# awkrail/svpc

Hardware: AMD Instinct MI355X
Metric: train steps/sec (vivt, batch=16, clip_seq=12) (higher is better)
Workload: dtype bf16x3; 1 GPU; MODEL_TYPE=vivt train step: N=16 videos/GPU x S=12 clips x Lv=100 frames x F=3072, Lt=22, D=768, H=12, L=6 (enc+step-enc+dec), V=951, A=384, E=10; dropout .1/.1/.4; fwd+bwd+allreduce+clip+BertAdam; mode=bf16x3, global_batch=16, parallelism=dp1, launch=hipGraph replay, gpus_requested=1

## Files before the change

include/svpc_hip.h:

```cpp
#ifndef SVPC_HIP_H
#define SVPC_HIP_H
#include <stddef.h>
#ifdef __cplusplus
extern "C" {
#endif

typedef struct ihipStream_t* svpc_stream_t;
typedef unsigned long long svpc_u64;

#define SVPC_ACT_NONE 0
#define SVPC_ACT_RELU 1
#define SVPC_ACT_GELU 2
#define SVPC_ACT_SIGMOID 3

const char* svpc_last_error(void);
int svpc_abi_version(void);

int svpc_ln_fwd(const float* x, const int* src_rows, const float* res, const float* gamma, const float* beta, float* y,
                float* mean, float* rstd, int R, int D, float eps, float p_pre, unsigned site_pre, float p_post,
                unsigned site_post, const svpc_u64* seed, const float* add1, int mod1, const float* add2, const int* idx2,
                svpc_stream_t stream);
int svpc_ln_fwd_t(const void* x, int x_dt, const int* src_rows, const void* res, const float* gamma, const float* beta, void* y,
                  int y_dt, float* mean, float* rstd, int R, int D, float eps, float p_pre, unsigned site_pre, float p_post,
                  unsigned site_post, const svpc_u64* seed, const float* add1, int mod1, const float* add2, const int* idx2,
// ... 67 lines not shown
int svpc_gemm_l32_preferred(int a_kc, int b_kc, int lda, int ldb, int M, int N, int K);
int svpc_gemm_l32(const float* A, int lda, int a_kc, const float* B, int ldb, int b_kc, float* C, int ldc, float* Z, int M, int N, int K,
                  const float* bias, int act, float p_drop, unsigned site, const svpc_u64* seed, int accumulate, float* workspace,
                  size_t workspace_bytes, svpc_stream_t stream);
int svpc_gemm_l32_r(const float* A, int lda, int a_kc, const float* B, int ldb, int b_kc, float* C, int ldc, float* Z, const float* R, int M,
                    int N, int K, const float* bias, int act, float p_drop, unsigned site, const svpc_u64* seed, int accumulate,
                    float* workspace, size_t workspace_bytes, svpc_stream_t stream);
int svpc_gemm_l32_rg(const float* A, int lda, int a_kc, const float* B, int ldb, int b_kc, float* C, int ldc, const float* R, const float* G,
                     int gact, int M, int N, int K, int accumulate, float* workspace, size_t workspace_bytes, svpc_stream_t stream);
int svpc_gemm_l32_x3(const float* A, int lda, int a_kc, const float* B, int ldb, int b_kc, float* C, int ldc, float* Z, const float* R, int M,
                     int N, int K, const float* bias, int act, float p_drop, unsigned site, const svpc_u64* seed, int accumulate,
                     float* workspace, size_t workspace_bytes, svpc_stream_t stream);
typedef struct svpc_gemm_problem { const float* A; const float* B; float* C; int M, N, K, lda, ldb, ldc; } svpc_gemm_problem;
int svpc_gemm_group(const svpc_gemm_problem* problems, int n, int a_kc, int b_kc, int accumulate, svpc_stream_t stream);
int svpc_gemm_group_x3(const svpc_gemm_problem* problems, int n, int a_kc, int b_kc, int accumulate, svpc_stream_t stream);
typedef struct svpc_wgrad_problem {
    const float* dz; const float* x; float* dw; float* db;
    int n_out, n_in, rows, ld_dz, ld_x, ld_dw;
} svpc_wgrad_problem;
int svpc_gemm_group_wgrad_max(void);
int svpc_gemm_group_wgrad_bf16_p8_ok(const void* problems, int n);
int svpc_gemm_group_wgrad_bf16_p8(const void* problems, int n, float* workspace, size_t workspace_bytes, svpc_stream_t stream);
int svpc_gemm_group_wgrad_bf16(const svpc_wgrad_problem* problems, int n, svpc_stream_t stream);
int svpc_gemm_group_wgrad_bf16_ws(const svpc_wgrad_problem* problems, int n, float* workspace, size_t workspace_bytes,
                                  svpc_stream_t stream);
int svpc_gemm_group_wgrad(const svpc_wgrad_problem* problems, int n, svpc_stream_t stream);
int svpc_act_bwd(const float* dy, const float* aux, float* dz, size_t n, int act, float p, unsigned site, const svpc_u64* seed,
                 svpc_stream_t stream);

int svpc_act_bwd_t(const void* dy, const void* aux, void* dz, int dt, size_t n, int act, float p, unsigned site, const svpc_u64* seed,
// ... 114 lines not shown
int svpc_ptr_mix_ce_bwd(const float* logits, const float* g, const float* pi, const int* labels, const int* row_c,
                        const int* row_vid, const int* csr_off, const int* csr_ent, const int* csr_id, const float* csr_w,
                        const float* P, const float* dP_ext, const float* dloss, float* dlogits, float* dg, float* dpi, int R, int V,
                        int c_max, int e_max, float smoothing, const float* row_w, svpc_stream_t stream);

int svpc_gumbel_noise(float* out, size_t n, unsigned site, const svpc_u64* seed, svpc_stream_t stream);
int svpc_gumbel_fwd(const float* P, const float* noise, const int* row_c, const float* emb, float* bow, int* idx, float* stats, int R,
                    int c_max, int V, int W, float tau, svpc_stream_t stream);
int svpc_gumbel_bwd(const float* P, const float* noise, const int* row_c, const float* stats, const float* dy, float* dP, int R,
                    int c_max, int V, float tau, svpc_stream_t stream);
int svpc_gumbel_emb_grad(const float* dbow, const int* idx, const float* stats, float* demb, int R, int V, int W,
                         svpc_stream_t stream);

int svpc_rownorm_fwd(const float* a, float* y, int R, int C, int mode, svpc_stream_t stream);
int svpc_rownorm_bwd(const float* dy, const float* y, const float* a, float* da, int R, int C, int mode, svpc_stream_t stream);
int svpc_span_mean_fwd(const float* x, const int* starts, const int* lens, const float* w, const float* add, const int* add_idx,
                       float* out, int G, int D, svpc_stream_t stream);
int svpc_span_mean_bwd(const float* dout, const int* starts, const int* lens, const float* w, float* dx, int G, int D,
                       svpc_stream_t stream);
int svpc_scatter_add_rows(const float* dx, const int* idx, float* dtable, int R, int D, int pad_row, svpc_stream_t stream);
int svpc_bce_rows_fwd(const float* p, const float* y, const int* widths, float* out, int R, int C, svpc_stream_t stream);
int svpc_bce_rows_bwd(const float* dout, const float* p, const float* y, const int* widths, float* dp, int R, int C,
                      svpc_stream_t stream);
int svpc_asl_rows_fwd(const float* p, const float* y, const float* active, float* out, int R, int C, float gneg, float gpos,
                      float clip, float eps, svpc_stream_t stream);
int svpc_asl_rows_bwd(const float* dout, const float* p, const float* y, const float* active, float* dp, int R, int C, float gneg,
                      float gpos, float clip, float eps, svpc_stream_t stream);
int svpc_loss_tail_ws_floats(int n_cap, int R);
int svpc_loss_tail_fwd(const float* cap_rows, int n_cap, const float* e_p, const float* align, const int* widths, int R, int Ce,
                       const float* a_p, const float* act, int Ca, const float* r_e, const float* r_a, float lambda, float gneg,
// ... 178 lines not shown
```

svpc_amd/csrc/elementwise.hip:

```cpp
#include "common.h"

template <typename T>
__global__ __launch_bounds__(256) void act_bwd_kernel(const T* __restrict__ dy, const T* __restrict__ aux,
                                                      T* __restrict__ dz, size_t n, int act, float p, uint32_t site,
                                                      const u64* __restrict__ seed_ptr) {
    const u64 seed = p > 0.f ? seed_ptr[0] : 0ull;
    const float ik = p > 0.f ? 1.0f / (1.0f - p) : 1.0f;
    for (size_t i = (size_t)blockIdx.x * 256 + threadIdx.x; i < n; i += (size_t)gridDim.x * 256) {
        float g = (float)dy[i];
        if (p > 0.f) g *= drop_scale(seed, site, i, p, ik);
        const float a = (float)aux[i];
        if (act == ACT_RELU) g = a > 0.f ? g : 0.f;
        else if (act == ACT_GELU) g *= gelu_erf_grad(a);
        else if (act == ACT_SIGMOID) g *= a * (1.0f - a);
        dz[i] = (T)g;
    }
}

__global__ __launch_bounds__(256) void act_bwd_bf16x8_kernel(const uint4* __restrict__ dy, const uint4* __restrict__ aux, uint4* __restrict__ dz,
                                                             size_t n8, int act, float p, uint32_t site, const u64* __restrict__ seed_ptr) {
    const u64 seed = p > 0.f ? seed_ptr[0] : 0ull;
    const float ik = p > 0.f ? 1.0f / (1.0f - p) : 1.0f;
    for (size_t q = (size_t)blockIdx.x * 256 + threadIdx.x; q < n8; q += (size_t)gridDim.x * 256) {
        const uint4 gv = dy[q], av = aux[q];
// ... 85 lines not shown
    }
}
__global__ __launch_bounds__(256) void rownorm_bwd_kernel(const float* __restrict__ dy, const float* __restrict__ y,
                                                          const float* __restrict__ a, float* __restrict__ da, int R, int C, int mode) {
    const int lane = threadIdx.x & 63, r = __builtin_amdgcn_readfirstlane(blockIdx.x * 4 + (threadIdx.x >> 6));
    if (r >= R) return;
    const size_t o = (size_t)r * C;
    float dot = 0.f, s = 0.f;
    for (int c = lane; c < C; c += 64) { dot += dy[o + c] * y[o + c]; if (mode == 0) s += a[o + c]; }
    dot = wave_sum(dot);
    if (mode == 0) {
        s = 1.0f / wave_sum(s);
        for (int c = lane; c < C; c += 64) da[o + c] = (dy[o + c] - dot) * s;
    } else {
        for (int c = lane; c < C; c += 64) da[o + c] = y[o + c] * (dy[o + c] - dot);
    }
}

__global__ __launch_bounds__(256) void span_mean_fwd_kernel(const float* __restrict__ x, const int* __restrict__ starts,
                                                            const int* __restrict__ lens, const float* __restrict__ w,
                                                            const float* __restrict__ add, const int* __restrict__ add_idx,
                                                            float* __restrict__ out, int G, int D) {
    const int g = blockIdx.x;
    const int s = starts[g], l = lens[g];
    for (int c = threadIdx.x; c < D; c += 256) {
        float acc = 0.f, wsum = 0.f;
        for (int r0 = 0; r0 < l; r0 += 8) {
            float xv[8], wv[8];
#pragma unroll
            for (int u = 0; u < 8; ++u) xv[u] = x[(size_t)(s + min(r0 + u, l - 1)) * D + c];
// ... 717 lines not shown
int svpc_fill_from(float* x, size_t n, const float* v, hipStream_t s) {
    if (n == 0) return 0;
    hipLaunchKernelGGL(fill_kernel, dim3(grid1d(n)), dim3(256), 0, s, x, n, v);
    return svpc_check_launch("fill_from");
}
int svpc_rownorm_fwd(const float* a, float* y, int R, int C, int mode, hipStream_t s) {
    if (R == 0) return 0;
    hipLaunchKernelGGL(rownorm_fwd_kernel, dim3(ceil_div(R, 4)), dim3(256), 0, s, a, y, R, C, mode);
    return svpc_check_launch("rownorm_fwd");
}
int svpc_rownorm_bwd(const float* dy, const float* y, const float* a, float* da, int R, int C, int mode, hipStream_t s) {
    if (R == 0) return 0;
    hipLaunchKernelGGL(rownorm_bwd_kernel, dim3(ceil_div(R, 4)), dim3(256), 0, s, dy, y, a, da, R, C, mode);
    return svpc_check_launch("rownorm_bwd");
}
int svpc_span_mean_fwd(const float* x, const int* starts, const int* lens, const float* w, const float* add, const int* add_idx,
                       float* out, int G, int D, hipStream_t s) {
    if (G == 0) return 0;
    hipLaunchKernelGGL(span_mean_fwd_kernel, dim3(G), dim3(256), 0, s, x, starts, lens, w, add, add_idx, out, G, D);
    return svpc_check_launch("span_mean_fwd");
}
int svpc_span_mean_bwd(const float* dout, const int* starts, const int* lens, const float* w, float* dx, int G, int D,
                       hipStream_t s) {
    if (G == 0) return 0;
    hipLaunchKernelGGL(span_mean_bwd_kernel, dim3(G), dim3(256), 0, s, dout, starts, lens, w, dx, G, D);
    return svpc_check_launch("span_mean_bwd");
}
int svpc_scatter_add_rows(const float* dx, const int* idx, float* dtable, int R, int D, int pad_row, hipStream_t s) {
    if (R == 0) return 0;
    hipLaunchKernelGGL(scatter_add_rows_kernel, dim3(R), dim3(256), 0, s, dx, idx, dtable, R, D, pad_row);
// ... 214 lines not shown
```

svpc_amd/csrc/gemm_l32.hip:

```cpp
#include "gemm_common.h"
#include <stdlib.h>

typedef __bf16 bf16x8 __attribute__((ext_vector_type(8)));
typedef const void __attribute__((address_space(1))) * l32_gptr;
typedef void __attribute__((address_space(3))) * l32_lptr;

constexpr int L32_BK = 32;
__device__ __attribute__((aligned(16))) const float l32_zeros[4] = {0.f, 0.f, 0.f, 0.f};

template <int N> __device__ __forceinline__ void l32_wait_vmcnt() { asm volatile("s_waitcnt vmcnt(%0)" ::"n"(N) : "memory"); }

template <int R, bool KC>
__device__ __forceinline__ const float* l32_src(const float* P, int ld, int m0, int rows, int k0, int j, int lane) {
    if (KC) {
        const int row = 8 * j + (lane >> 3), pos = lane & 7;
        const int c = pos ^ ((row >> 1) & 7);
        const int gr = min(m0 + row, rows - 1);
        return P + (size_t)gr * ld + k0 + 4 * c;
    } else {
        constexpr int CPR = R / 4;
        const int krow = j * (64 / CPR) + lane / CPR, c = lane % CPR;
        const int gm = min(m0 + 4 * c, rows - 4);
        return P + (size_t)(k0 + krow) * ld + gm;
    }
// ... 407 lines not shown

template <bool A_KC, bool B_KC, bool X3 = false>
static int gemm_group_go(const GemmGroupArgs& g, int tiles, hipStream_t stream) {
    constexpr int LDS = 4 * 2 * 2 * 64 * L32_BK * 4;
    static bool attr_set = false;
    if (!attr_set) {
        hipError_t e = hipFuncSetAttribute(reinterpret_cast<const void*>(&gemm_group_kernel<A_KC, B_KC, X3>),
                                           hipFuncAttributeMaxDynamicSharedMemorySize, LDS);
        if (e != hipSuccess) { svpc_set_error("gemm_group: cannot raise the dynamic LDS limit"); return (int)e; }
        attr_set = true;
    }
    hipLaunchKernelGGL((gemm_group_kernel<A_KC, B_KC, X3>), dim3(tiles), dim3(256), LDS, stream, g);
    return svpc_check_launch("gemm_group");
}

template <bool B_KC, int NW, bool X3 = false>
__device__ __forceinline__ void skinny_partials(float (*part)[16][64], const float* __restrict__ arow, const float* __restrict__ brow,
                                                int ldb, int K) {
    constexpr int BATCH = NW == 8 ? 10 : 12;
    const int lane = threadIdx.x & 63, wave = __builtin_amdgcn_readfirstlane(threadIdx.x >> 6);
    const int nsteps = K >> 4;
    floatx16 acc;
#pragma unroll
    for (int e = 0; e < 16; ++e) acc[e] = 0.f;
    for (int s0 = wave; s0 < nsteps; s0 += NW * BATCH) {
        float4 av[BATCH][2];
        float bv[BATCH][8];
#pragma unroll
        for (int u = 0; u < BATCH; ++u) {
            const int s = min(s0 + NW * u, nsteps - 1);
            const float* ap = arow + 16 * s;
            av[u][0] = *reinterpret_cast<const float4*>(ap);
            av[u][1] = *reinterpret_cast<const float4*>(ap + 4);
            if (B_KC) {
                const float* bp = brow + 16 * s;
                const float4 b0 = *reinterpret_cast<const float4*>(bp), b1 = *reinterpret_cast<const float4*>(bp + 4);
                bv[u][0] = b0.x; bv[u][1] = b0.y; bv[u][2] = b0.z; bv[u][3] = b0.w;
                bv[u][4] = b1.x; bv[u][5] = b1.y; bv[u][6] = b1.z; bv[u][7] = b1.w;
            } else {
                const float* bp = brow + (size_t)(16 * s) * ldb;
#pragma unroll
                for (int j = 0; j < 8; ++j) bv[u][j] = bp[(size_t)j * ldb];
            }
        }
#pragma unroll
        for (int u = 0; u < BATCH; ++u) {
            const int s = s0 + NW * u;
            if (s < nsteps) {
// ... 52 lines not shown
                                                          float* __restrict__ C, int ldc, int M, int N, int K, Epi epi, int tiles_n, int ts) {
    __shared__ float part[4][16][64];
    const int tm = blockIdx.x / tiles_n, tn = blockIdx.x - tm * tiles_n;
    skinny_tile<B_KC, 4, X3>(part, A, lda, B, ldb, C, ldc, M, N, K, epi, tm, tn, ts);
}
template <int NW, bool X3 = false, bool B_KC = true>
__global__ __launch_bounds__(64 * NW) void gemm_group_skinny_kernel(GemmGroupArgs g) {
    __shared__ float part[NW][16][64];
    int pi = 0;
    while (pi + 1 < g.n && (int)blockIdx.x >= g.p[pi + 1].tile0) ++pi;
    const GemmProb& q = g.p[pi];
    const int tile = blockIdx.x - q.tile0;
    const int tm = tile / q.tiles_n, tn = tile - tm * q.tiles_n;
    Epi epi{nullptr, ACT_NONE, 0.f, 0u, nullptr, g.accumulate, nullptr};
    skinny_tile<B_KC, NW, X3>(part, q.A, q.lda, q.B, q.ldb, q.C, q.ldc, q.M, q.N, q.K, epi, tm, tn);
}

struct LstmStep {
    const float* h_prev[2]; const float* c_prev[2]; const float* w_hh[2]; const float* gx[2]; const int* rows[2]; const float* active;
    float* h[2]; float* c[2]; float* gates[2]; int N, D;
};
template <bool X3>
__global__ __launch_bounds__(256) void lstm_pair_step_fwd_kernel(LstmStep a) {
    __shared__ float part[4][16][64];
    const int z = blockIdx.y, u0 = blockIdx.x * 8, m0 = blockIdx.z * 32;
    const int lane = threadIdx.x & 63, r = lane & 31, hh = lane >> 5;
    const int N = a.N, D = a.D;
    const float* arow = a.h_prev[z] + (size_t)min(m0 + r, N - 1) * D + 8 * hh;
    const float* brow = a.w_hh[z] + (size_t)((r >> 3) * D + u0 + (r & 7)) * D + 8 * hh;
    const int row = threadIdx.x >> 3, j = threadIdx.x & 7, n = m0 + row;
// ... 64 lines not shown
    if (!a_kc && (M % 4 != 0)) return 0;
    if (!b_kc && (N % 4 != 0)) return 0;
    return 1;
}

int svpc_gemm_l32_preferred(int a_kc, int b_kc, int lda, int ldb, int M, int N, int K) {
    if (!svpc_gemm_l32_supported(a_kc, b_kc, lda, ldb, M, N, K)) return 0;
    const int t128 = ceil_div(M, 128) * ceil_div(N, 128), t64 = ceil_div(M, 64) * ceil_div(N, 64);
    static int env_w = -1;
    if (env_w < 0) { const char* e = getenv("SVPC_L32_WAVESPLIT"); env_w = e ? atoi(e) : 1; }
    if (K % L32_BK != 0) return (t128 <= 300) ? 1 : 0;
    if (env_w && t64 <= 256 && K >= 4 * L32_BK && t64 * 4 >= 32) return 1;
    return (t128 <= 300 && K < 2048) ? 1 : 0;
}

struct HostWgradProblem { const float* dz; const float* x; float* dw; float* db; int n_out, n_in, rows, ld_dz, ld_x, ld_dw; };

int svpc_gemm_group_wgrad_max(void) { return GROUP_MAX; }

static int gemm_group_x(const void* problems, int n, int a_kc, int b_kc, int accumulate, int x3, hipStream_t stream) {
    if (n == 0) return 0;
    SVPC_REQUIRE(n > 0 && n <= GEMM_GROUP_MAX, "gemm_group: 1..32 problems per launch");
    const HostGemmProblem* hp = reinterpret_cast<const HostGemmProblem*>(problems);
    GemmGroupArgs g{};
    g.n = n; g.accumulate = accumulate;
    int tiles = 0;
    static int env_skinny = -1;
    if (env_skinny < 0) { const char* e = getenv("SVPC_L32_SKINNY"); env_skinny = e ? atoi(e) : 1; }
    bool skinny = env_skinny && a_kc;
    if (!b_kc && x3) skinny = false;
// ... 105 lines not shown
                           workspace_bytes, stream);
}
}
static int gemm_l32_x(const float* A, int lda, int a_kc, const float* B, int ldb, int b_kc, float* C, int ldc, float* Z, const float* R,
                      const float* G, int gact, int M, int N, int K, const float* bias, int act, float p_drop, unsigned site, const u64* seed,
                      int accumulate, float* workspace, size_t workspace_bytes, int x3, hipStream_t stream) {
    if (M == 0 || N == 0) return 0;
    SVPC_REQUIRE(svpc_gemm_l32_supported(a_kc, b_kc, lda, ldb, M, N, K) && ((((uintptr_t)A) | ((uintptr_t)B)) & 15) == 0,
                 "gemm_l32: needs K % 32 == 0 (or both operands k-contiguous and K % 4 == 0) and 16-byte aligned fp32 rows");
    SVPC_REQUIRE(p_drop <= 0.f || seed != nullptr, "gemm: dropout needs a seed pointer");
    Epi epi{bias, act, p_drop, site, seed, accumulate, Z, R, G, gact};
    static int env_tile = -1, env_split = -1;
    const int remap = gemm_remap_env();
    if (env_tile < 0) { const char* e = getenv("SVPC_L32_TILE"); env_tile = e ? atoi(e) : 0; }
    if (env_split < 0) { const char* e = getenv("SVPC_L32_SPLITK"); env_split = e ? atoi(e) : 0; }
    static int env_skinny = -1;
    if (env_skinny < 0) { const char* e = getenv("SVPC_L32_SKINNY"); env_skinny = e ? atoi(e) : 1; }
    static int skinny_m = -1;
    if (skinny_m < 0) { const char* e = getenv("SVPC_L32_SKINNY_M"); skinny_m = e ? atoi(e) : 256; }
    if (env_skinny && a_kc && M <= skinny_m && N >= 32 && (K & 15) == 0 && (lda & 3) == 0 && (!b_kc || (ldb & 3) == 0)) {
        static int env_ts = -1;
        if (env_ts < 0) { const char* e = getenv("SVPC_L32_SKINNY_TS"); env_ts = e ? atoi(e) : 24; }
        const int t24 = ceil_div(M, 24) * ceil_div(N, 24), t32 = ceil_div(M, 32) * ceil_div(N, 32);
        const int ts = (env_ts == 24 && t24 <= 256 && t32 < t24 && t32 > 64) ? 24 : 32;
        const int tn_ = ceil_div(N, ts);
        dim3 grids(ceil_div(M, ts) * tn_);
        if (x3) {
            if (b_kc) hipLaunchKernelGGL((gemm_skinny_kernel<true, true>), grids, dim3(256), 0, stream, A, lda, B, ldb, C, ldc, M, N, K, epi, tn_, ts);
            else hipLaunchKernelGGL((gemm_skinny_kernel<false, true>), grids, dim3(256), 0, stream, A, lda, B, ldb, C, ldc, M, N, K, epi, tn_, ts);
        } else if (b_kc) hipLaunchKernelGGL((gemm_skinny_kernel<true, false>), grids, dim3(256), 0, stream, A, lda, B, ldb, C, ldc, M, N, K, epi, tn_, ts);
        else hipLaunchKernelGGL((gemm_skinny_kernel<false, false>), grids, dim3(256), 0, stream, A, lda, B, ldb, C, ldc, M, N, K, epi, tn_, ts);
        return svpc_check_launch("gemm_skinny");
    }
    const int t128 = ceil_div(M, 128) * ceil_div(N, 128), t64 = ceil_div(M, 64) * ceil_div(N, 64);
    int mode = (M >= 96 && N >= 96 && t128 > 300) ? 128 : 65;
// ... 57 lines not shown
```

svpc_amd/grad_tail.py:

```python
from __future__ import annotations

import ctypes
import os

import torch

from . import _lib

USE_GROUPED_WGRAD = os.environ.get("SVPC_NO_GROUPED_WGRAD", "") == ""
GROUP_BF16 = os.environ.get("SVPC_NO_GROUP_BF16", "") == ""
GROUP_FLUSH_AT = int(os.environ.get("SVPC_GROUP_FLUSH_AT", "16"))
GROUP_MAX_TILES = int(os.environ.get("SVPC_GROUP_MAX_TILES", "1200"))
COLSUM_FLUSH_AT = 48

_WQ16 = []
_WQ = []
_CQ = []
_FQ = []
_JOIN_QUEUED = [False]
GRAD_READY_HOOK = None
HOOKS_PAUSED = [0]
_OPS = []


# ... 60 lines not shown
    _WQ16.append((dz, x, wgrad, bgrad))
    _queue_end_of_backward_join()
    return True


def defer_wgrad(dz, x, wgrad, bgrad):
    o = _ops()
    if USE_GROUPED_WGRAD and GROUP_BF16 and o._fast() and wgrad is not None and dz.dtype == torch.bfloat16 and x.dtype == torch.bfloat16:
        return _defer_wgrad16(dz, x, wgrad, bgrad)
    if not (USE_GROUPED_WGRAD and o._fast() and wgrad is not None and dz.dtype == torch.float32 and x.dtype == torch.float32) or o.BWD_EXACT:
        return False
    rows, n_out = dz.shape
    n_in = x.shape[1]
    if rows < 1 or n_out % 4 or n_in % 4 or dz.stride(0) % 4 or x.stride(0) % 4 or wgrad.stride(0) % 4:
        return False
    if (dz.data_ptr() | x.data_ptr()) % 16 or dz.stride(1) != 1 or x.stride(1) != 1 or not wgrad.is_contiguous():
        return False
    tiles = -(-n_out // 64) * -(-n_in // 64)
    if tiles > GROUP_MAX_TILES:
        return False
    wp = wgrad.data_ptr()
    if any(q[2].data_ptr() == wp for q in _WQ):
        flush_wgrads(bf16=False)
    _WQ.append((dz, x, wgrad, bgrad))
    if len(_WQ) >= min(GROUP_FLUSH_AT, _lib.load().svpc_gemm_group_wgrad_max()):
        flush_wgrads(bf16=False)
    _queue_end_of_backward_join()
    return True


def _problem_table(queue):
# ... 117 lines not shown
```

svpc_amd/graph.py:

```python
from __future__ import annotations

import gc

import torch


_STREAMS = {}


class capturing:

    def __init__(self, graph, light=False, **kw):
        self.light = bool(light)
        if self.light:
            self.graph = graph
            self.pool = kw.get("pool")
            self.stream = kw.get("stream") or torch.cuda.current_stream()
            self.mode = kw.get("capture_error_mode", "global")
            self.stream_ctx = torch.cuda.stream(self.stream)
        else:
            self.cm = torch.cuda.graph(graph, **kw)

    def __enter__(self):
        self.was = gc.isenabled()
# ... 61 lines not shown
        if exchange is not None:
            exchange.start_early()
        cut[0].backward(cut[1].grad)
        model.split_boundary = None


class GraphedTrainStep:
    def __init__(self, model, optimizer, forward_args, warmup=2, exchange=None):
        self.model, self.opt, self.args = model, optimizer, forward_args
        self.exchange = exchange
        assert optimizer.arena is not None, "run at least one eager step first (the gradient arena is built lazily)"
        gc.collect()
        cur = torch.cuda.current_stream()
        self.stream = cur if cur != torch.cuda.default_stream() else ops_stream()
        self.stream.wait_stream(cur)
        with torch.cuda.stream(self.stream):
            for _ in range(warmup):
                self._eager()
        cur.wait_stream(self.stream)
        torch.cuda.synchronize()
        gc.collect()
        unit_grad(torch.empty((), dtype=torch.float32, device=next(model.parameters()).device))
        self.graph = torch.cuda.CUDAGraph()
        self.graph_opt = None
        if exchange is None:
            with capturing(self.graph, stream=self.stream):
                optimizer.zero_grad()
                self.loss = model(*forward_args)[0]
                self.loss.backward(unit_grad(self.loss))
                optimizer.launch()
        else:
            from . import ops
            model.split_backward = True
            with capturing(self.graph, stream=self.stream, capture_error_mode="thread_local"):
                optimizer.zero_grad()
                self.loss = model(*forward_args)[0]
                self.loss.backward(unit_grad(self.loss))
                ops.join_side()
            self.graph_clip = torch.cuda.CUDAGraph()
            with capturing(self.graph_clip, pool=self.graph.pool(), stream=self.stream, capture_error_mode="thread_local"):
                out, cut = model.split_boundary
                out.backward(cut.grad)
                ops.join_side()
            self.graph_opt = torch.cuda.CUDAGraph()
            with capturing(self.graph_opt, pool=self.graph.pool(), stream=self.stream, capture_error_mode="thread_local"):
                optimizer.launch()
        self._versions = optimizer.weights.versions()

    def _eager(self):
# ... 27 lines not shown
```

svpc_amd/model.py:

```python
from __future__ import annotations

import math

import numpy as np
import torch
import torch.nn as nn

from . import ops
from .ops_common import ACT_GELU, ACT_NONE, ACT_RELU, ACT_SIGMOID, BulkUpload, FIdx, Idx

PAD_ROW = 0


def _sinusoid(max_len, d):
    pe = torch.zeros(max_len, d)
    pos = torch.arange(0, max_len).float().unsqueeze(1)
    div = torch.exp(torch.arange(0, d, 2).float() * -(math.log(10000.0) / d))
    pe[:, 0::2] = torch.sin(pos * div)
    pe[:, 1::2] = torch.cos(pos * div)
    return pe


def _i32(v, device):
    return torch.tensor(v, dtype=torch.int32, device=device)
# ... 442 lines not shown
        self.W2 = nn.Linear(D + A, D)
        self.W3 = nn.Linear(D, 3)
        self.W4 = nn.Linear(W, 1)

    def set_pretrained_embedding(self, pretrained_embedding, freeze):
        emb = nn.Embedding.from_pretrained(pretrained_embedding, freeze=freeze)
        self.action_embeddings = emb.weight

    def verb_table(self):
        ae = self.action_embeddings
        if isinstance(ae, nn.Embedding):
            raise TypeError("unsupported operand type(s) for @: 'Tensor' and 'Embedding' — call "
                            "set_pretrained_embedding first (reference behaviour, model.py:798)")
        return ae

    def run(self, g, ents, plan_sim, cx):
        sel = self.action_selector
        hid = ops.linear(g, getattr(sel, "0").weight, getattr(sel, "0").bias, act=ACT_RELU, drop=cx.drop(0.4))
        a = ops.linear(hid, getattr(sel, "3").weight, getattr(sel, "3").bias, act=ACT_SIGMOID)
        fbar = ops.linear(ops.row_normalize(a), self.verb_table(), None, trans_w=True)
        hat_h = ops.linear(g, self.W1[0].weight, self.W1[0].bias, act=ACT_RELU)
        q = ops.linear(torch.cat([hat_h, a], 1), self.W2.weight, self.W2.bias)
        heads = ops.sim_heads(hat_h, fbar, self.W3.weight, self.W3.bias, self.W4.weight, self.W4.bias)
        if heads is not None:
            c, w4f = heads
        else:
            c = ops.softmax_rows(ops.linear(hat_h, self.W3.weight, self.W3.bias))
            w4f = ops.linear(fbar, self.W4.weight, self.W4.bias).reshape(-1)
        e, ebar, eall = ops.sim_recur(q, c, w4f, ents, *plan_sim)
        return e, a, ebar, eall, fbar

    def forward(self, video_vectors, entity_vectors):
        g = video_vectors.squeeze(0).contiguous()
        S, E = g.shape[0], entity_vectors.shape[0]
        cx = _Ctx(self.config, self.training, ops.default_rng(g.device))
        e, a, ebar, eall, fbar = self.run(g, entity_vectors.contiguous(),
                                          (Idx([0]), Idx([S]), Idx([0]), Idx([E]), E), cx)
# ... 458 lines not shown
            act_t = torch.cat(list(actions), 0)
            r_e = r_a = None
            if mode == "full":
                noise = None
                if self.gumbel_noise is not None:
                    noise = self._pad_cat([n.reshape(-1, n.shape[-1]) for n in self.gumbel_noise], c_max)
                    if pack is not None:
                        noise = torch.index_select(noise, 0, pack.full_rows64)
                bow = ops.gumbel_bow(P, row_c, self.text_embeddings.word_embeddings.weight, cfg.temperature,
                                     noise=noise, rng=cx.rng, site=cx.rng.site())
                if pack is not None:
                    pooled = ops.span_mean(bow, pack.off_idx, pack.len_idx)
                else:
                    pooled = ops.span_mean(bow, plan.text_starts, plan.text_lens, weights=text_mask)
                seq_vec = self._bilstm(pooled, plan)
                r_e, r_a, _, r_all, _ = self.recipe_reasoner.run(seq_vec, ents, plan.sim, cx)
            total = ops.loss_tail(cap_rows, e_p, a_p, r_e, r_a, align, act_t, plan.step_ne, cfg.lambda_ if mode == "full" else 0.0)

        if pack is not None:
            P = ops.scatter_rows(P, pack.full_rows64, T * Lt, inv=pack.inv_rows)
        prediction_scores_list = []
        for b in range(N):
            o, n = plan.h_step_off[b], plan.h_step_len[b]
            prediction_scores_list.append(P[o * Lt:(o + n) * Lt, :c_list[b]].reshape(n, Lt, c_list[b]))
            if sim_out is not None:
                E_b = plan.h_ent_len[b]
                ent_list.append(e_p[o:o + n, :E_b])
                act_list.append(a_p[o:o + n])
                if predict:
                    md = {"entity_probs": ent_list[-1], "action_probs": act_list[-1],
                          "entity_vectors": [ents[plan.h_ent_off[b]:plan.h_ent_off[b] + E_b], eall[o:o + n, :E_b]]}
# ... 61 lines not shown
```

svpc_amd/ops.py:

```python
from __future__ import annotations

import ctypes
import math
import numbers
import os
import struct

import torch
from torch.autograd import Function as _TorchFunction

from . import _lib
from .ops_common import ACT_GELU, ACT_NONE, ACT_RELU, ACT_SIGMOID, FIdx, Idx, SeqInfo, as_idx
from .grad_tail import (HOOKS_PAUSED, _WgradProblem, _queue_end_of_backward_join, _ready, bias_grad, defer_colsum,
                        defer_finalize, defer_partials, defer_wgrad, flush_finalizes, flush_pending, flush_wgrads, hooks_paused, join_side)

_WS = {}
_WS_BYTES = 256 << 20


_DEV_IDX = [None]


def _stream():
    i = _DEV_IDX[0]
# ... 1398 lines not shown
        for tgt, val in zip(ctx.direct, outs):
            if tgt is not None:
                tgt.add_(val.view_as(tgt)); res.append(None)
            else:
                res.append(val)
        return (dhh, dfb) + tuple(res)


def sim_heads(hh, fb, W3, b3, W4, b4):
    if (not hh.is_cuda or hh.dtype != torch.float32 or fb.dtype != torch.float32 or tuple(W3.shape) != (3, hh.shape[1]) or
            tuple(W4.shape) != (1, fb.shape[1]) or hh.shape[1] > 1024 or fb.shape[1] > 512 or b3 is None or b4 is None):
        return None
    return _SimHeads.apply(hh, fb, W3, b3, W4, b4)


class _PtrAttn(Function):
    @staticmethod
    def forward(ctx, dec, proj, bank, step_ne, lt):
        _need_gpu(dec)
        dec, proj, bank = _c(dec), _c(proj), _c(bank)
        T, e_max, D = bank.shape
        dev = dec.device
        ne = step_ne.dev(dev)
        pi = torch.empty(T * lt, e_max, dtype=torch.float32, device=dev)
        att = torch.empty(T * lt, D, dtype=torch.float32, device=dev)
        _lib.call("ptr_attn_fwd", _p(dec), _p(proj), _p(bank), _p(ne), _p(pi), _p(att), T, lt, e_max, D, _stream())
        ctx.save_for_backward(dec, proj, bank, ne, pi)
        ctx.cfg = (T, lt, e_max, D)
        ctx.set_materialize_grads(False)
        return pi, att
# ... 1891 lines not shown
```

Before: 92.20 steps/s (one step = 16 clip-sequences per GPU; whole-job aggregate).

## Fuse the simulator front-end linear chain into grouped skinny GEMM launches

Adds a fused skinny-GEMM kernel that runs up to four problems per launch. It folds bias, activation, dropout, residual add and activation-gradient epilogues into the GEMM, and can read A from two sources so no concat is needed. The action-selector and simulator front end become a custom autograd function that uses these launches. It also uses a fused rownorm-backward plus add plus sigmoid-grad kernel and splits W2's weight gradient into two deferred wgrads. The aim is fewer small kernel launches and intermediate tensors on small M, at the cost of much more code and possible bitwise differences.

```diff
diff --git a/include/svpc_hip.h b/include/svpc_hip.h
--- a/include/svpc_hip.h
+++ b/include/svpc_hip.h
@@ -105,6 +105,13 @@
 typedef struct svpc_gemm_problem { const float* A; const float* B; float* C; int M, N, K, lda, ldb, ldc; } svpc_gemm_problem;
 int svpc_gemm_group(const svpc_gemm_problem* problems, int n, int a_kc, int b_kc, int accumulate, svpc_stream_t stream);
 int svpc_gemm_group_x3(const svpc_gemm_problem* problems, int n, int a_kc, int b_kc, int accumulate, svpc_stream_t stream);
+typedef struct svpc_fused_problem {
+    const float* A; const float* A2; const float* B; float* C; const float* bias; const float* R; const float* G;
+    int M, N, K, ksplit, lda, lda2, ldb, ldc, act; float p_drop; unsigned site; int gact; float g_p; unsigned g_site;
+} svpc_fused_problem;
+int svpc_gemm_skinny_fused_max(void);
+int svpc_gemm_l32_is_skinny(int a_kc, int b_kc, int lda, int ldb, int M, int N, int K);
+int svpc_gemm_skinny_fused(const svpc_fused_problem* problems, int n, int b_kc, int x3, const svpc_u64* seed, svpc_stream_t stream);
 typedef struct svpc_wgrad_problem {
     const float* dz; const float* x; float* dw; float* db;
     int n_out, n_in, rows, ld_dz, ld_x, ld_dw;
@@ -249,6 +256,8 @@
 
 int svpc_rownorm_fwd(const float* a, float* y, int R, int C, int mode, svpc_stream_t stream);
 int svpc_rownorm_bwd(const float* dy, const float* y, const float* a, float* da, int R, int C, int mode, svpc_stream_t stream);
+int svpc_rownorm_bwd_add_act(const float* dy, const float* y, const float* a, const float* add, const float* aux, int gact, float* da, int R,
+                             int C, int mode, svpc_stream_t stream);
 int svpc_span_mean_fwd(const float* x, const int* starts, const int* lens, const float* w, const float* add, const int* add_idx,
                        float* out, int G, int D, svpc_stream_t stream);
 int svpc_span_mean_bwd(const float* dout, const int* starts, const int* lens, const float* w, float* dx, int G, int D,
diff --git a/svpc_amd/csrc/elementwise.hip b/svpc_amd/csrc/elementwise.hip
--- a/svpc_amd/csrc/elementwise.hip
+++ b/svpc_amd/csrc/elementwise.hip
@@ -123,6 +123,28 @@
         for (int c = lane; c < C; c += 64) da[o + c] = (dy[o + c] - dot) * s;
     } else {
         for (int c = lane; c < C; c += 64) da[o + c] = y[o + c] * (dy[o + c] - dot);
+    }
+}
+__global__ __launch_bounds__(256) void rownorm_bwd_add_act_kernel(const float* __restrict__ dy, const float* __restrict__ y,
+                                                                  const float* __restrict__ a, const float* __restrict__ add,
+                                                                  const float* __restrict__ aux, int gact, float* __restrict__ da, int R,
+                                                                  int C, int mode) {
+    const int lane = threadIdx.x & 63, r = __builtin_amdgcn_readfirstlane(blockIdx.x * 4 + (threadIdx.x >> 6));
+    if (r >= R) return;
+    const size_t o = (size_t)r * C;
+    float dot = 0.f, s = 0.f;
+    for (int c = lane; c < C; c += 64) { dot += dy[o + c] * y[o + c]; if (mode == 0) s += a[o + c]; }
+    dot = wave_sum(dot);
+    if (mode == 0) s = 1.0f / wave_sum(s);
+    for (int c = lane; c < C; c += 64) {
+#pragma clang fp contract(off)
+        const float d = mode == 0 ? (dy[o + c] - dot) * s : y[o + c] * (dy[o + c] - dot);
+        float g = add ? add[o + c] + d : d;
+        const float x = aux[o + c];
+        if (gact == ACT_RELU) g = x > 0.f ? g : 0.f;
+        else if (gact == ACT_GELU) g *= gelu_erf_grad(x);
+        else if (gact == ACT_SIGMOID) g *= x * (1.0f - x);
+        da[o + c] = g;
     }
 }
 
@@ -870,6 +892,13 @@
     hipLaunchKernelGGL(rownorm_bwd_kernel, dim3(ceil_div(R, 4)), dim3(256), 0, s, dy, y, a, da, R, C, mode);
     return svpc_check_launch("rownorm_bwd");
 }
+int svpc_rownorm_bwd_add_act(const float* dy, const float* y, const float* a, const float* add, const float* aux, int gact, float* da, int R,
+                             int C, int mode, hipStream_t s) {
+    if (R == 0) return 0;
+    SVPC_REQUIRE(aux != nullptr, "rownorm_bwd_add_act: needs what the activation's forward kept");
+    hipLaunchKernelGGL(rownorm_bwd_add_act_kernel, dim3(ceil_div(R, 4)), dim3(256), 0, s, dy, y, a, add, aux, gact, da, R, C, mode);
+    return svpc_check_launch("rownorm_bwd_add_act");
+}
 int svpc_span_mean_fwd(const float* x, const int* starts, const int* lens, const float* w, const float* add, const int* add_idx,
                        float* out, int G, int D, hipStream_t s) {
     if (G == 0) return 0;
diff --git a/svpc_amd/csrc/gemm_l32.hip b/svpc_amd/csrc/gemm_l32.hip
--- a/svpc_amd/csrc/gemm_l32.hip
+++ b/svpc_amd/csrc/gemm_l32.hip
@@ -445,9 +445,9 @@
     return svpc_check_launch("gemm_group");
 }
 
-template <bool B_KC, int NW, bool X3 = false>
+template <bool B_KC, int NW, bool X3 = false, bool A2SRC = false>
 __device__ __forceinline__ void skinny_partials(float (*part)[16][64], const float* __restrict__ arow, const float* __restrict__ brow,
-                                                int ldb, int K) {
+                                                int ldb, int K, const float* __restrict__ arow2 = nullptr, int ksplit = 0) {
     constexpr int BATCH = NW == 8 ? 10 : 12;
     const int lane = threadIdx.x & 63, wave = __builtin_amdgcn_readfirstlane(threadIdx.x >> 6);
     const int nsteps = K >> 4;
@@ -460,9 +460,15 @@
 #pragma unroll
         for (int u = 0; u < BATCH; ++u) {
             const int s = min(s0 + NW * u, nsteps - 1);
-            const float* ap = arow + 16 * s;
-            av[u][0] = *reinterpret_cast<const float4*>(ap);
-            av[u][1] = *reinterpret_cast<const float4*>(ap + 4);
+            if constexpr (A2SRC) {
+                const int k0 = 16 * s + 8 * (lane >> 5);
+                av[u][0] = *reinterpret_cast<const float4*>(k0 < ksplit ? arow + 16 * s : arow2 + (16 * s - ksplit));
+                av[u][1] = *reinterpret_cast<const float4*>(k0 + 4 < ksplit ? arow + 16 * s + 4 : arow2 + (16 * s + 4 - ksplit));
+            } else {
+                const float* ap = arow + 16 * s;
+                av[u][0] = *reinterpret_cast<const float4*>(ap);
+                av[u][1] = *reinterpret_cast<const float4*>(ap + 4);
+            }
             if (B_KC) {
                 const float* bp = brow + 16 * s;
                 const float4 b0 = *reinterpret_cast<const float4*>(bp), b1 = *reinterpret_cast<const float4*>(bp + 4);
@@ -545,6 +551,68 @@
     const int tm = tile / q.tiles_n, tn = tile - tm * q.tiles_n;
     Epi epi{nullptr, ACT_NONE, 0.f, 0u, nullptr, g.accumulate, nullptr};
     skinny_tile<B_KC, NW, X3>(part, q.A, q.lda, q.B, q.ldb, q.C, q.ldc, q.M, q.N, q.K, epi, tm, tn);
+}
+
+struct FusedProb {
+    const float* A; const float* A2; const float* B; float* C; const float* bias; const float* R; const float* G;
+    int M, N, K, ksplit, lda, lda2, ldb, ldc, act; float p_drop; unsigned site; int gact; float g_p; unsigned g_site;
+    int tile0, tiles_n;
+};
+constexpr int FUSED_MAX = 4;
+struct FusedArgs { int n; const u64* seed; FusedProb p[FUSED_MAX]; };
+
+template <bool B_KC, bool X3>
+__global__ __launch_bounds__(256) void gemm_skinny_fused_kernel(FusedArgs g) {
+#pragma clang fp contract(off)
+    __shared__ float part[4][16][64];
+    int pi = 0;
+    while (pi + 1 < g.n && (int)blockIdx.x >= g.p[pi + 1].tile0) ++pi;
+    const FusedProb& q = g.p[pi];
+    const int tile = blockIdx.x - q.tile0;
+    const int tm = tile / q.tiles_n, tn = tile - tm * q.tiles_n;
+    const int lane = threadIdx.x & 63;
+    const int m0 = tm * 32, n0 = tn * 32;
+    const int r = lane & 31, h = lane >> 5;
+    const int am = min(m0 + r, q.M - 1), bcol = min(n0 + r, q.N - 1);
+    const float* __restrict__ arow = q.A + (size_t)am * q.lda + 8 * h;
+    const float* __restrict__ brow = B_KC ? q.B + (size_t)bcol * q.ldb + 8 * h : q.B + (size_t)(8 * h) * q.ldb + bcol;
+    if (q.A2) skinny_partials<B_KC, 4, X3, true>(part, arow, brow, q.ldb, q.K, q.A2 + (size_t)am * q.lda2 + 8 * h, q.ksplit);
+    else skinny_partials<B_KC, 4, X3>(part, arow, brow, q.ldb, q.K);
+    const bool any_drop = q.p_drop > 0.f || q.g_p > 0.f;
+    const u64 seed = any_drop ? g.seed[0] : 0ull;
+    const float inv_keep = q.p_drop > 0.f ? 1.0f / (1.0f - q.p_drop) : 1.0f;
+    const float g_inv_keep = q.g_p > 0.f ? 1.0f / (1.0f - q.g_p) : 1.0f;
+    const int col = threadIdx.x & 31;
+    float vs[4], bs[4], rv[4], gv[4]; size_t os[4]; bool oks[4];
+#pragma unroll
+    for (int i = 0; i < 4; ++i) {
+        const int row = (threadIdx.x >> 5) + 8 * i;
+        const int e = (row & 3) + 4 * (row >> 3), l = col + 32 * ((row >> 2) & 1);
+        float v = part[0][e][l];
+#pragma unroll
+        for (int w = 1; w < 4; ++w) v += part[w][e][l];
+        vs[i] = v;
+        oks[i] = m0 + row < q.M && n0 + col < q.N;
+        const int cr = min(m0 + row, q.M - 1), cc = min(n0 + col, q.N - 1);
+        os[i] = (size_t)cr * q.ldc + cc;
+        bs[i] = q.bias ? q.bias[cc] : 0.f;
+        rv[i] = q.R ? q.R[os[i]] : 0.f;
+        gv[i] = q.G ? q.G[os[i]] : 0.f;
+    }
+#pragma unroll
+    for (int i = 0; i < 4; ++i) {
+        float t = apply_act(vs[i] + bs[i], q.act);
+        if (q.p_drop > 0.f) t *= drop_scale(seed, q.site, os[i], q.p_drop, inv_keep);
+        float v = (t + 0.f) + rv[i];
+        if (q.G) {
+            if (q.g_p > 0.f) v *= drop_scale(seed, q.g_site, os[i], q.g_p, g_inv_keep);
+            const float a = gv[i];
+            if (q.gact == ACT_RELU) v = a > 0.f ? v : 0.f;
+            else if (q.gact == ACT_GELU) v *= gelu_erf_grad(a);
+            else if (q.gact == ACT_SIGMOID) v *= a * (1.0f - a);
+        }
+        if (oks[i]) q.C[os[i]] = v;
+    }
 }
 
 struct LstmStep {
@@ -639,6 +707,52 @@
     return (t128 <= 300 && K < 2048) ? 1 : 0;
 }
 
+int svpc_gemm_l32_is_skinny(int a_kc, int b_kc, int lda, int ldb, int M, int N, int K) {
+    static int env_skinny = -1, skinny_m = -1;
+    if (env_skinny < 0) { const char* e = getenv("SVPC_L32_SKINNY"); env_skinny = e ? atoi(e) : 1; }
+    if (skinny_m < 0) { const char* e = getenv("SVPC_L32_SKINNY_M"); skinny_m = e ? atoi(e) : 256; }
+    if (!svpc_gemm_l32_supported(a_kc, b_kc, lda, ldb, M, N, K)) return 0;
+    return (env_skinny && a_kc && M <= skinny_m && N >= 32 && (K & 15) == 0 && (lda & 3) == 0 && (!b_kc || (ldb & 3) == 0)) ? 1 : 0;
+}
+
+struct HostFusedProblem {
+    const float* A; const float* A2; const float* B; float* C; const float* bias; const float* R; const float* G;
+    int M, N, K, ksplit, lda, lda2, ldb, ldc, act; float p_drop; unsigned site; int gact; float g_p; unsigned g_site;
+};
+int svpc_gemm_skinny_fused_max(void) { return FUSED_MAX; }
+int svpc_gemm_skinny_fused(const void* problems, int n, int b_kc, int x3, const u64* seed, hipStream_t stream) {
+    if (n == 0) return 0;
+    SVPC_REQUIRE(n > 0 && n <= FUSED_MAX, "gemm_skinny_fused: 1..4 problems per launch");
+    const HostFusedProblem* hp = reinterpret_cast<const HostFusedProblem*>(problems);
+    FusedArgs g{};
+    g.n = n; g.seed = seed;
+    int tiles = 0;
+    for (int i = 0; i < n; ++i) {
+        const HostFusedProblem& h = hp[i];
+        if (h.M == 0 || h.N == 0) { SVPC_REQUIRE(n == 1, "gemm_skinny_fused: an empty problem only on its own"); return 0; }
+        SVPC_REQUIRE(svpc_gemm_l32_is_skinny(1, b_kc, h.lda, h.ldb, h.M, h.N, h.K) && ((((uintptr_t)h.A) | ((uintptr_t)h.B)) & 15) == 0,
+                     "gemm_skinny_fused: every problem must be a skinny one (M <= 256, N >= 32, K % 16 == 0, 16-byte aligned fp32 rows)");
+        SVPC_REQUIRE(h.A2 == nullptr || (h.ksplit > 0 && h.ksplit < h.K && (h.ksplit & 3) == 0 && (h.lda2 & 3) == 0 && h.lda >= h.ksplit &&
+                                         h.lda2 >= h.K - h.ksplit && (((uintptr_t)h.A2) & 15) == 0),
+                     "gemm_skinny_fused: a second A source needs 0 < ksplit < K, ksplit % 4 == 0 and 16-byte aligned rows wide enough");
+        SVPC_REQUIRE(h.A2 != nullptr || h.lda >= h.K, "gemm_skinny_fused: lda < K");
+        SVPC_REQUIRE(h.ldc >= h.N && (b_kc ? h.ldb >= h.K : h.ldb >= h.N), "gemm_skinny_fused: leading dimension below the row width");
+        SVPC_REQUIRE((h.p_drop <= 0.f && h.g_p <= 0.f) || seed != nullptr, "gemm_skinny_fused: dropout needs a seed pointer");
+        SVPC_REQUIRE(h.g_p <= 0.f || h.G != nullptr, "gemm_skinny_fused: the backward of a dropout needs the activation it followed (G)");
+        SVPC_REQUIRE(!(x3 && !b_kc), "gemm_skinny_fused: bf16x3 products only with a k-contiguous B");
+        FusedProb& q = g.p[i];
+        q.A = h.A; q.A2 = h.A2; q.B = h.B; q.C = h.C; q.bias = h.bias; q.R = h.R; q.G = h.G;
+        q.M = h.M; q.N = h.N; q.K = h.K; q.ksplit = h.ksplit; q.lda = h.lda; q.lda2 = h.lda2; q.ldb = h.ldb; q.ldc = h.ldc; q.act = h.act;
+        q.p_drop = h.p_drop; q.site = h.site; q.gact = h.gact; q.g_p = h.g_p; q.g_site = h.g_site;
+        q.tile0 = tiles; q.tiles_n = ceil_div(h.N, 32);
+        tiles += ceil_div(h.M, 32) * q.tiles_n;
+    }
+    if (x3) hipLaunchKernelGGL((gemm_skinny_fused_kernel<true, true>), dim3(tiles), dim3(256), 0, stream, g);
+    else if (b_kc) hipLaunchKernelGGL((gemm_skinny_fused_kernel<true, false>), dim3(tiles), dim3(256), 0, stream, g);
+    else hipLaunchKernelGGL((gemm_skinny_fused_kernel<false, false>), dim3(tiles), dim3(256), 0, stream, g);
+    return svpc_check_launch("gemm_skinny_fused");
+}
+
 struct HostWgradProblem { const float* dz; const float* x; float* dw; float* db; int n_out, n_in, rows, ld_dz, ld_x, ld_dw; };
 
 int svpc_gemm_group_wgrad_max(void) { return GROUP_MAX; }
@@ -774,11 +888,7 @@
     const int remap = gemm_remap_env();
     if (env_tile < 0) { const char* e = getenv("SVPC_L32_TILE"); env_tile = e ? atoi(e) : 0; }
     if (env_split < 0) { const char* e = getenv("SVPC_L32_SPLITK"); env_split = e ? atoi(e) : 0; }
-    static int env_skinny = -1;
-    if (env_skinny < 0) { const char* e = getenv("SVPC_L32_SKINNY"); env_skinny = e ? atoi(e) : 1; }
-    static int skinny_m = -1;
-    if (skinny_m < 0) { const char* e = getenv("SVPC_L32_SKINNY_M"); skinny_m = e ? atoi(e) : 256; }
-    if (env_skinny && a_kc && M <= skinny_m && N >= 32 && (K & 15) == 0 && (lda & 3) == 0 && (!b_kc || (ldb & 3) == 0)) {
+    if (svpc_gemm_l32_is_skinny(a_kc, b_kc, lda, ldb, M, N, K)) {
         static int env_ts = -1;
         if (env_ts < 0) { const char* e = getenv("SVPC_L32_SKINNY_TS"); env_ts = e ? atoi(e) : 24; }
         const int t24 = ceil_div(M, 24) * ceil_div(N, 24), t32 = ceil_div(M, 32) * ceil_div(N, 32);
diff --git a/svpc_amd/grad_tail.py b/svpc_amd/grad_tail.py
--- a/svpc_amd/grad_tail.py
+++ b/svpc_amd/grad_tail.py
@@ -98,7 +98,8 @@
     n_in = x.shape[1]
     if rows < 1 or n_out % 4 or n_in % 4 or dz.stride(0) % 4 or x.stride(0) % 4 or wgrad.stride(0) % 4:
         return False
-    if (dz.data_ptr() | x.data_ptr()) % 16 or dz.stride(1) != 1 or x.stride(1) != 1 or not wgrad.is_contiguous():
+    cols_of = wgrad.dim() == 2 and wgrad.stride(1) == 1 and tuple(wgrad.shape) == (n_out, n_in)
+    if (dz.data_ptr() | x.data_ptr()) % 16 or dz.stride(1) != 1 or x.stride(1) != 1 or not (wgrad.is_contiguous() or cols_of):
         return False
     tiles = -(-n_out // 64) * -(-n_in // 64)
     if tiles > GROUP_MAX_TILES:
diff --git a/svpc_amd/graph.py b/svpc_amd/graph.py
--- a/svpc_amd/graph.py
+++ b/svpc_amd/graph.py
@@ -99,7 +99,8 @@
         cur = torch.cuda.current_stream()
         self.stream = cur if cur != torch.cuda.default_stream() else ops_stream()
         self.stream.wait_stream(cur)
-        with torch.cuda.stream(self.stream):
+        from . import ops
+        with torch.cuda.stream(self.stream), ops.chain_fusion():
             for _ in range(warmup):
                 self._eager()
         cur.wait_stream(self.stream)
@@ -109,15 +110,14 @@
         self.graph = torch.cuda.CUDAGraph()
         self.graph_opt = None
         if exchange is None:
-            with capturing(self.graph, stream=self.stream):
+            with capturing(self.graph, stream=self.stream), ops.chain_fusion():
                 optimizer.zero_grad()
                 self.loss = model(*forward_args)[0]
                 self.loss.backward(unit_grad(self.loss))
                 optimizer.launch()
         else:
-            from . import ops
             model.split_backward = True
-            with capturing(self.graph, stream=self.stream, capture_error_mode="thread_local"):
+            with capturing(self.graph, stream=self.stream, capture_error_mode="thread_local"), ops.chain_fusion():
                 optimizer.zero_grad()
                 self.loss = model(*forward_args)[0]
                 self.loss.backward(unit_grad(self.loss))
diff --git a/svpc_amd/model.py b/svpc_amd/model.py
--- a/svpc_amd/model.py
+++ b/svpc_amd/model.py
@@ -480,13 +480,21 @@
                             "set_pretrained_embedding first (reference behaviour, model.py:798)")
         return ae
 
-    def run(self, g, ents, plan_sim, cx):
+    def run(self, g, ents, plan_sim, cx, g_shared=True):
         sel = self.action_selector
-        hid = ops.linear(g, getattr(sel, "0").weight, getattr(sel, "0").bias, act=ACT_RELU, drop=cx.drop(0.4))
-        a = ops.linear(hid, getattr(sel, "3").weight, getattr(sel, "3").bias, act=ACT_SIGMOID)
-        fbar = ops.linear(ops.row_normalize(a), self.verb_table(), None, trans_w=True)
-        hat_h = ops.linear(g, self.W1[0].weight, self.W1[0].bias, act=ACT_RELU)
-        q = ops.linear(torch.cat([hat_h, a], 1), self.W2.weight, self.W2.bias)
+        drop = cx.drop(0.4)
+        front = getattr(ops, "sim_front", None)
+        front = front and front(g, getattr(sel, "0").weight, getattr(sel, "0").bias, getattr(sel, "3").weight, getattr(sel, "3").bias,
+                                self.verb_table(), self.W1[0].weight, self.W1[0].bias, self.W2.weight, self.W2.bias, drop=drop,
+                                g_shared=g_shared)
+        if front:
+            a, fbar, hat_h, q = front
+        else:
+            hid = ops.linear(g, getattr(sel, "0").weight, getattr(sel, "0").bias, act=ACT_RELU, drop=drop)
+            a = ops.linear(hid, getattr(sel, "3").weight, getattr(sel, "3").bias, act=ACT_SIGMOID)
+            fbar = ops.linear(ops.row_normalize(a), self.verb_table(), None, trans_w=True)
+            hat_h = ops.linear(g, self.W1[0].weight, self.W1[0].bias, act=ACT_RELU)
+            q = ops.linear(torch.cat([hat_h, a], 1), self.W2.weight, self.W2.bias)
         heads = ops.sim_heads(hat_h, fbar, self.W3.weight, self.W3.bias, self.W4.weight, self.W4.bias)
         if heads is not None:
             c, w4f = heads
@@ -975,7 +983,7 @@
                 else:
                     pooled = ops.span_mean(bow, plan.text_starts, plan.text_lens, weights=text_mask)
                 seq_vec = self._bilstm(pooled, plan)
-                r_e, r_a, _, r_all, _ = self.recipe_reasoner.run(seq_vec, ents, plan.sim, cx)
+                r_e, r_a, _, r_all, _ = self.recipe_reasoner.run(seq_vec, ents, plan.sim, cx, g_shared=False)
             total = ops.loss_tail(cap_rows, e_p, a_p, r_e, r_a, align, act_t, plan.step_ne, cfg.lambda_ if mode == "full" else 0.0)
 
         if pack is not None:
diff --git a/svpc_amd/ops.py b/svpc_amd/ops.py
--- a/svpc_amd/ops.py
+++ b/svpc_amd/ops.py
@@ -1436,6 +1436,194 @@
     return _SimHeads.apply(hh, fb, W3, b3, W4, b4)
 
 
+CHAIN_FUSION = os.environ.get("SVPC_NO_CHAIN_FUSION", "") == ""
+_CHAIN_SCOPE = [0]
+FUSED_STATS = [0, 0]
+
+
+class chain_fusion:
+
+    def __enter__(self):
+        _CHAIN_SCOPE[0] += 1
+        return self
+
+    def __exit__(self, *exc):
+        _CHAIN_SCOPE[0] -= 1
+        return False
+
+
+class _FusedProblem(ctypes.Structure):
+    _fields_ = [("A", ctypes.c_void_p), ("A2", ctypes.c_void_p), ("B", ctypes.c_void_p), ("C", ctypes.c_void_p), ("bias", ctypes.c_void_p),
+                ("R", ctypes.c_void_p), ("G", ctypes.c_void_p), ("M", ctypes.c_int), ("N", ctypes.c_int), ("K", ctypes.c_int),
+                ("ksplit", ctypes.c_int), ("lda", ctypes.c_int), ("lda2", ctypes.c_int), ("ldb", ctypes.c_int), ("ldc", ctypes.c_int),
+                ("act", ctypes.c_int), ("p_drop", ctypes.c_float), ("site", ctypes.c_uint), ("gact", ctypes.c_int), ("g_p", ctypes.c_float),
+                ("g_site", ctypes.c_uint)]
+
+
+def _fused_problem(A, b_ptr, ldb, C, N, K, A2=None, bias=None, act=ACT_NONE, p=0.0, site=0, R=None, G=None, gact=ACT_NONE, g_p=0.0,
+                   g_site=0):
+    for t in (R, G):
+        assert t is None or (t.dtype == torch.float32 and t.shape == C.shape and t.stride() == C.stride())
+    return _FusedProblem(A.data_ptr(), _p(A2), b_ptr, C.data_ptr(), _p(bias), _p(R), _p(G), C.shape[0], N, K,
+                         A.shape[1] if A2 is not None else 0, A.stride(0), A2.stride(0) if A2 is not None else 0, ldb, C.stride(0), int(act),
+                         float(p), int(site), int(gact), float(g_p), int(g_site))
+
+
+def _fused_launch(probs, b_kc, x3, seed):
+    arr = (_FusedProblem * len(probs))(*probs)
+    _lib.call("gemm_skinny_fused", ctypes.addressof(arr), len(probs), int(b_kc), int(bool(x3)), _p(seed), _stream())
+    FUSED_STATS[0] += 1
+
+
+def _skinny_route(ptrs, b_kc, lda, ldb, M, N, K, x3=False):
+    lib = _lib.load()
+    if M <= 0 or any(p % 16 for p in ptrs) or lib.svpc_gemm_l32_is_skinny(1, b_kc, lda, ldb, M, N, K) != 1:
+        return False
+    if x3:
+        return True
+    return _fast() and USE_L32 and not BWD_EXACT and lib.svpc_gemm_l32_preferred(1, b_kc, lda, ldb, M, N, K) == 1
+
+
+def _fp32_param_grads(dz, x, w, has_b, direct, trans_w, need_w, need_b):
+    wgrad, bgrad = direct
+    N, K = dz.shape[1], x.shape[1]
+    dw = db = None
+    if wgrad is not None and not trans_w and (not has_b or bgrad is not None):
+        if defer_wgrad(dz, x, wgrad, bgrad if has_b else None):
+            return None, None
+    if wgrad is not None or need_w:
+        acc = 1 if wgrad is not None else 0
+        dw = wgrad if wgrad is not None else torch.empty_like(w)
+        if trans_w:
+            _gemm(x, x.stride(0), 0, dz, N, 0, dw, K, N, dz.shape[0], accumulate=acc)
+        else:
+            _gemm(dz, N, 0, x, x.stride(0), 0, dw, N, K, dz.shape[0], accumulate=acc)
+        if wgrad is not None:
+            _ready(wgrad, "w")
+            dw = None
+    if has_b and (bgrad is not None or need_b):
+        if bgrad is not None:
+            bias_grad(dz, bgrad)
+        else:
+            db = _colsum(dz).view(-1)
+    return dw, db
+
+
+def _act_bwd(dy, aux, act, p=0.0, site=0, seed=None):
+    dz = torch.empty_like(dy)
+    _lib.call("act_bwd_t", _p(dy), _p(aux), _p(dz), 0, dy.numel(), int(act), float(p), int(site), _p(seed), _stream())
+    FUSED_STATS[1] += 1
+    return dz
+
+
+class _SimFront(Function):
+
+    @staticmethod
+    def forward(ctx, g, g2, w0, b0, w3, b3, verb, w1, b1, w2, b2, drop):
+        _need_gpu(g)
+        g, w0, w3, verb, w1, w2 = _c(g), _c(w0), _c(w3), _c(verb), _c(w1), _c(w2)
+        M, D = g.shape
+        A, Wd = w3.shape[0], verb.shape[1]
+        dev = g.device
+        x3 = is_x3()
+        p, site, seed = _drop_args(drop)
+        new = lambda n: torch.empty(M, n, dtype=torch.float32, device=dev)
+        hid, hat_h, a, an, fbar, q = new(D), new(D), new(A), new(A), new(Wd), new(D)
+        if _skinny_route((g.data_ptr(), w0.data_ptr(), w1.data_ptr()), 1, D, D, M, D, D, x3):
+            _fused_launch([_fused_problem(g, w0.data_ptr(), D, hid, D, D, bias=b0, act=ACT_RELU, p=p, site=site),
+                           _fused_problem(g, w1.data_ptr(), D, hat_h, D, D, bias=b1, act=ACT_RELU)], 1, x3, seed)
+        else:
+            _gemm(g, D, 1, w0, D, 1, hid, M, D, D, bias=b0, act=ACT_RELU, p=p, site=site, seed=seed, x3=x3)
+            _gemm(g, D, 1, w1, D, 1, hat_h, M, D, D, bias=b1, act=ACT_RELU, x3=x3)
+            FUSED_STATS[1] += 1
+        _gemm(hid, D, 1, w3, D, 1, a, M, A, D, bias=b3, act=ACT_SIGMOID, x3=x3)
+        _lib.call("rownorm_fwd", _p(a), _p(an), M, A, 0, _stream())
+        _gemm(an, A, 1, verb, Wd, 0, fbar, M, Wd, A, x3=x3)
+        if D % 4 == 0 and A % 4 == 0 and _skinny_route((hat_h.data_ptr(), a.data_ptr(), w2.data_ptr()), 1, D + A, D + A, M, D, D + A, x3):
+            _fused_launch([_fused_problem(hat_h, w2.data_ptr(), D + A, q, D, D + A, A2=a, bias=b2)], 1, x3, None)
+        else:
+            cat = torch.cat([hat_h, a], 1)
+            _gemm(cat, D + A, 1, w2, D + A, 1, q, M, D, D + A, bias=b2, x3=x3)
+            FUSED_STATS[1] += 1
+        ctx.save_for_backward(g, w0, w3, verb, w1, w2, hid, a, an, hat_h, seed)
+        ctx.cfg = (p, site, g2 is not None, b0 is not None, b3 is not None, b1 is not None, b2 is not None)
+        ctx.direct = tuple((_direct(w), _direct(b) if b is not None else None) for w, b in ((w0, b0), (w3, b3), (verb, None), (w1, b1), (w2, b2)))
+        return a, fbar, hat_h, q
+
+    @staticmethod
+    def backward(ctx, da, dfbar, dhh, dq):
+        g, w0, w3, verb, w1, w2, hid, a, an, hat_h, seed = ctx.saved_tensors
+        p, site, shared, has_b0, has_b3, has_b1, has_b2 = ctx.cfg
+        d0, d3, dv, d1, d2 = ctx.direct
+        need = ctx.needs_input_grad
+        M, D = g.shape
+        A, Wd = a.shape[1], verb.shape[1]
+        dev = g.device
+        da, dfbar, dhh, dq = _c(da), _c(dfbar), _c(dhh), _c(dq)
+        new = lambda n: torch.empty(M, n, dtype=torch.float32, device=dev)
+        dzh, da1 = new(D), new(A)
+        if (D % 4 == 0 and A % 4 == 0 and _skinny_route((dq.data_ptr(), w2.data_ptr()), 0, D, D + A, M, D + A, D)
+                and _lib.load().svpc_gemm_l32_is_skinny(1, 0, D, D + A, M, D, D) == 1
+                and _lib.load().svpc_gemm_l32_is_skinny(1, 0, D, D + A, M, A, D) == 1):
+            _fused_launch([_fused_problem(dq, w2.data_ptr(), D + A, dzh, D, D, R=dhh, G=hat_h, gact=ACT_RELU),
+                           _fused_problem(dq, w2.data_ptr() + 4 * D, D + A, da1, A, D, R=da)], 0, False, None)
+        else:
+            dcat = new(D + A)
+            _gemm(dq, D, 1, w2, D + A, 0, dcat, M, D + A, D)
+            dzh = _act_bwd(torch.add(dhh, dcat[:, :D]), hat_h, ACT_RELU)
+            da1 = torch.add(da, dcat[:, D:])
+        dw2 = db2 = None
+        if need[9] or need[10] or d2[0] is not None:
+            w2g, b2g = d2
+            two = (D % 4 == 0 and A % 4 == 0 and w2g is not None and (not has_b2 or b2g is not None)
+                   and defer_wgrad(dq, hat_h, w2g[:, :D], b2g if has_b2 else None))
+            if two:
+                if not defer_wgrad(dq, a, w2g[:, D:], None):
+                    raise _lib.SvpcKernelError("sim_front: the second column range of W2's gradient was refused by the grouped launch")
+            else:
+                dw2, db2 = _fp32_param_grads(dq, torch.cat([hat_h, a], 1), w2, has_b2, d2, False, need[9], need[10])
+        dg1 = None
+        if need[0] or need[1]:
+            dg1 = new(D)
+            _gemm(dzh, D, 1, w1, D, 0, dg1, M, D, D)
+        dw1, db1 = _fp32_param_grads(dzh, g, w1, has_b1, d1, False, need[7], need[8])
+        dan = new(A)
+        _gemm(dfbar, Wd, 1, verb, Wd, 1, dan, M, A, Wd)
+        dverb, _ = _fp32_param_grads(dfbar, an, verb, False, dv, True, need[6], False)
+        dz3 = new(A)
+        _lib.call("rownorm_bwd_add_act", _p(dan), _p(an), _p(a), _p(da1), _p(a), ACT_SIGMOID, _p(dz3), M, A, 0, _stream())
+        FUSED_STATS[0] += 1
+        dzhid = new(D)
+        if _skinny_route((dz3.data_ptr(), w3.data_ptr()), 0, A, D, M, D, A):
+            _fused_launch([_fused_problem(dz3, w3.data_ptr(), D, dzhid, D, A, G=hid, gact=ACT_RELU, g_p=p, g_site=site)], 0, False, seed)
+        else:
+            dhid = new(D)
+            _gemm(dz3, A, 1, w3, D, 0, dhid, M, D, A)
+            dzhid = _act_bwd(dhid, hid, ACT_RELU, p, site, seed)
+        dw3, db3 = _fp32_param_grads(dz3, hid, w3, has_b3, d3, False, need[4], need[5])
+        dg2 = None
+        if need[0] or need[1]:
+            dg2 = new(D)
+            if not shared and _skinny_route((dzhid.data_ptr(), w0.data_ptr()), 0, D, D, M, D, D):
+                _fused_launch([_fused_problem(dzhid, w0.data_ptr(), D, dg2, D, D, R=dg1)], 0, False, None)
+                dg1 = None
+            else:
+                _gemm(dzhid, D, 1, w0, D, 0, dg2, M, D, D)
+                if not shared:
+                    dg2, dg1 = torch.add(dg1, dg2), None
+        dw0, db0 = _fp32_param_grads(dzhid, g, w0, has_b0, d0, False, need[2], need[3])
+        if shared:
+            return dg1, dg2, dw0, db0, dw3, db3, dverb, dw1, db1, dw2, db2, None
+        return dg2, None, dw0, db0, dw3, db3, dverb, dw1, db1, dw2, db2, None
+
+
+def sim_front(g, w0, b0, w3, b3, verb, w1, b1, w2, b2, drop=None, g_shared=True):
+    if not (CHAIN_FUSION and _CHAIN_SCOPE[0] > 0 and _fast() and USE_L32 and not BWD_EXACT and g.is_cuda and g.dim() == 2 and all(t.dtype == torch.float32 for t in (g, w0, w3, verb, w1, w2))
+            and all(t is not None for t in (b0, b3, b1, b2)) and w2.shape[1] == w1.shape[0] + w3.shape[0] and g.shape[0] > 0):
+        return None
+    return _SimFront.apply(g, g if g_shared else None, w0, b0, w3, b3, verb, w1, b1, w2, b2, drop)
+
+
 class _PtrAttn(Function):
     @staticmethod
     def forward(ctx, dec, proj, bank, step_ne, lt):
```

New measurement: 92.39 steps/s (one step = 16 clip-sequences per GPU; whole-job aggregate), median of 6. No clear change (+0.2%).
